# tracel-ai/cubecl

Measured on NVIDIA H100. Metric: bf16_matmul_tflops, higher is better.
Workload: dtype bf16

## Files before the change

cubecl_b200/csrc/gemm_wgmma.cu:

```cuda
#include <cuda_bf16.h>
#include <cuda_fp16.h>

#include "kernel_params.h"
#include "ptx.cuh"

using namespace b200;

enum : int { KIND_F16 = 0, KIND_BF16 = 1, KIND_TF32 = 2, KIND_E4M3 = 3, KIND_E5M2 = 4, KIND_U8 = 5, KIND_S8 = 6 };
enum : int { OUT_F16 = 0, OUT_BF16 = 1, OUT_F32 = 2 };

constexpr int kNumThreads = 384;

#include <type_traits>
struct TileCoord {
  uint32_t b, m_blk, n_blk;
};

__device__ __forceinline__ TileCoord tile_coord(uint32_t t, const GemmParams& p) {
  const uint32_t per_batch = p.tiles_m * p.tiles_n;
  TileCoord c;
  c.b = t / per_batch;
  uint32_t r = t - c.b * per_batch;
  const uint32_t strip = p.group_m * p.tiles_n;
  const uint32_t g = r / strip;
  const uint32_t first_m = g * p.group_m;
  const uint32_t gsize = min(p.group_m, p.tiles_m - first_m);
  const uint32_t in = r - g * strip;
  c.m_blk = first_m + in % gsize;
  c.n_blk = in / gsize;
  return c;
}

struct WorkUnit {
  uint32_t tile, kb0, kb1;
  uint32_t slab;
  bool partial;
};

struct UnitIter {
  uint32_t c, C, num_kb;
  uint32_t r;
  uint32_t u;
  uint64_t pos, hi;
  uint32_t next_tile;
  bool open;
};

__device__ __forceinline__ UnitIter unit_iter(uint32_t cluster, uint32_t n_clusters, uint32_t num_kb) {
  UnitIter it;
  it.c = cluster; it.C = n_clusters; it.num_kb = num_kb;
  it.r = cluster; it.u = 0; it.pos = 0; it.hi = 0; it.next_tile = cluster; it.open = false;
  return it;
}

__device__ __forceinline__ uint64_t sk_range_lo(uint32_t r, const GemmParams& p, uint32_t num_kb) {
  return (static_cast<uint64_t>(r) * p.sk_tiles * num_kb) / p.sk_ranges;
}
__device__ __forceinline__ uint32_t sk_owner(uint64_t x, const GemmParams& p, uint32_t num_kb) {
  return static_cast<uint32_t>(((x + 1) * p.sk_ranges - 1) / (static_cast<uint64_t>(p.sk_tiles) * num_kb));
}

__device__ __forceinline__ bool next_unit(UnitIter& it, const GemmParams& p, WorkUnit& w) {
  while (p.sk_tiles != 0 && it.r < p.sk_ranges) {
    if (!it.open) {
      it.pos = sk_range_lo(it.r, p, it.num_kb);
      it.hi = sk_range_lo(it.r + 1, p, it.num_kb);
      it.u = 0;
      it.open = true;
    }
    if (it.pos < it.hi) {
      const uint32_t tau = static_cast<uint32_t>(it.pos / it.num_kb);
      const uint64_t t0 = static_cast<uint64_t>(tau) * it.num_kb;
      const uint64_t end = (it.hi < t0 + it.num_kb) ? it.hi : t0 + it.num_kb;
      w.tile = p.full_tiles + tau;
      w.kb0 = static_cast<uint32_t>(it.pos - t0);
      w.kb1 = static_cast<uint32_t>(end - t0);
      w.partial = !(w.kb0 == 0 && w.kb1 == it.num_kb);
      w.slab = it.r * p.sk_umax + it.u;
      it.pos = end;
      ++it.u;
      return true;
    }
    it.r += it.C;
    it.open = false;
  }
  if (it.next_tile < p.full_tiles) {
    w.tile = it.next_tile; w.kb0 = 0; w.kb1 = it.num_kb; w.slab = 0; w.partial = false;
    it.next_tile += it.C;
    return true;
  }
  return false;
}


template <int OUT>
__device__ __forceinline__ void store_pair(uint64_t row_ptr, uint32_t n, uint32_t N, bool vec, uint32_t v0, uint32_t v1) {
  if constexpr (OUT == OUT_F32) {
    uint32_t* dst = reinterpret_cast<uint32_t*>(row_ptr) + n;
    if (vec && n + 1 < N) *reinterpret_cast<uint2*>(dst) = make_uint2(v0, v1);
    else { if (n < N) dst[0] = v0; if (n + 1 < N) dst[1] = v1; }
  } else {
    uint16_t* dst = reinterpret_cast<uint16_t*>(row_ptr) + n;
    uint32_t packed;
    if constexpr (OUT == OUT_BF16) asm("cvt.rn.bf16x2.f32 %0, %1, %2;" : "=r"(packed) : "r"(v1), "r"(v0));
    else asm("cvt.rn.f16x2.f32 %0, %1, %2;" : "=r"(packed) : "r"(v1), "r"(v0));
    if (vec && n + 1 < N) *reinterpret_cast<uint32_t*>(dst) = packed;
    else { if (n < N) dst[0] = static_cast<uint16_t>(packed & 0xFFFFu); if (n + 1 < N) dst[1] = static_cast<uint16_t>(packed >> 16); }
  }
}

__device__ __forceinline__ uint32_t acc_bits(float x) { return __float_as_uint(x); }
__device__ __forceinline__ uint32_t acc_bits(uint32_t x) { return x; }

enum : int { QM_NONE = 0, QM_BLOCK = 1, QM_TENSOR = 2 };
enum : int { CB_NONE = 0, CB_DGRAD = 1, CB_WGRAD = 2 };
template <int CG, int BLOCK_N, bool A_MN, bool B_MN, int KIND, int OUT, int STAGES, bool PROMOTE = false, int MT = 1, int QM = QM_NONE,
          bool CONV = false, int CB = CB_NONE>
__device__ __forceinline__ void gemm_body(const CUtensorMap* tma_a_hi, const CUtensorMap* tma_b_hi, const CUtensorMap* tma_a_lo,
                                          const CUtensorMap* tma_b_lo, const CUtensorMap* tma_out, const GemmParams& p) {
  constexpr bool INT_ACC = (KIND == KIND_U8 || KIND == KIND_S8) && QM != QM_BLOCK;
  static_assert(QM == QM_NONE || (KIND == KIND_S8 && !A_MN && !B_MN && !PROMOTE && MT == 1), "quantized operands: s8, K-major");
  static_assert(!CONV || ((KIND == KIND_BF16 || KIND == KIND_F16) && !A_MN && !B_MN && !PROMOTE && MT == 1 && QM == QM_NONE),
                "convolution: 16-bit kinds, K-major operands");
  static_assert(CB != CB_DGRAD || CONV, "data gradient: the convolution producer");
  static_assert(CB != CB_WGRAD || (!CONV && A_MN && B_MN && (KIND == KIND_BF16 || KIND == KIND_F16) && !PROMOTE && MT == 1 && QM == QM_NONE),
                "weight gradient: 16-bit kinds, MN-major operands");
  constexpr uint32_t SC_A_BYTES = (QM == QM_BLOCK) ? 128u * 4u * 4u : 0u;
  constexpr uint32_t SC_STAGE_BYTES = (QM == QM_BLOCK) ? SC_A_BYTES + BLOCK_N * 4u * 4u : 0u;
  constexpr int ESZ = (KIND == KIND_TF32) ? 4 : (KIND >= KIND_E4M3) ? 1 : 2;
  static_assert(ESZ == 2 || (!A_MN && !B_MN), "wgmma reads MN-major operands for 16-bit kinds only");
  constexpr int BLOCK_K = 128 / ESZ;
  constexpr int MMA_K = 32 / ESZ;
  constexpr int N_LOCAL = BLOCK_N / CG;
  constexpr uint32_t A_SUB_BYTES = 128 * 128;
  constexpr uint32_t A_BYTES = MT * A_SUB_BYTES;
  constexpr uint32_t B_BYTES = BLOCK_N * 128;
  constexpr uint32_t STAGE_BYTES = A_BYTES + B_BYTES;
  constexpr int CHUNK_N = 64;
  constexpr uint32_t CHUNK_BYTES = BLOCK_K * 128;
  constexpr int NUM_CHUNKS = N_LOCAL / CHUNK_N;
  constexpr int NACC = BLOCK_N / 2;
  static_assert(STAGE_BYTES % 1024 == 0, "stages must keep 1024-byte alignment for SWIZZLE_128B");
  using Acc = typename std::conditional<INT_ACC, uint32_t, float>::type;
  static_assert(!PROMOTE || (KIND == KIND_BF16 && !A_MN && !B_MN && MT == 1), "promoted accumulation: bf16, K-major operands");
  static_assert(MT == 1 || (MT == 2 && ESZ == 2), "two M sub-tiles per CTA: 16-bit kinds");
  constexpr int PH = (BLOCK_N % 128 == 0) ? 128 : 112;
  static_assert(!PROMOTE || BLOCK_N % PH == 0, "promoted partials tile BLOCK_N");
  constexpr int CW = (OUT == OUT_F32) ? 32 : 64;

  extern __shared__ uint8_t smem_raw[];
  const uint32_t smem_base = (smem_u32(smem_raw) + 1023u) & ~1023u;
  const uint32_t sc_base = smem_base + STAGES * STAGE_BYTES;
  const uint32_t bar_base = sc_base + STAGES * SC_STAGE_BYTES;
  auto full_bar = [&](int s) { return bar_base + 8u * s; };
  auto empty_bar = [&](int s) { return bar_base + 8u * (STAGES + s); };
  const uint32_t split_flag = bar_base + 16u * STAGES;
  const uint32_t epi_base = bar_base + 1024u;

  const uint32_t wg = threadIdx.x >> 7;
  const uint32_t rank = (CG == 2) ? cluster_ctarank() : 0u;
  const uint32_t cluster_id = (CG == 2) ? cluster_id_x() : blockIdx.x;
  const uint32_t n_clusters = (CG == 2) ? num_clusters_x() : gridDim.x;

  if (threadIdx.x == 0) {
    tma_prefetch_desc(tma_a_hi);
    tma_prefetch_desc(tma_b_hi);
    if (p.k_segments > 1) { tma_prefetch_desc(tma_a_lo); tma_prefetch_desc(tma_b_lo); }
    if constexpr (QM == QM_BLOCK) { tma_prefetch_desc(tma_a_lo); tma_prefetch_desc(tma_b_lo); }
    if (p.tma_store) tma_prefetch_desc(tma_out);
    for (int s = 0; s < STAGES; ++s) {
      mbar_init(full_bar(s), 1);
      mbar_init(empty_bar(s), 2 * CG);
    }
    fence_mbar_init();
  }
  if constexpr (CG == 2) cluster_sync_all(); else __syncthreads();

  const uint32_t seg_kb = (p.K + BLOCK_K - 1) / BLOCK_K;
  const bool hyb = (KIND == KIND_TF32) && p.hyb != 0 && p.k_segments == 3;
  const uint32_t seg_kb1 = hyb ? (p.K + 63u) / 64u : seg_kb;
  const uint32_t num_kb = (p.k_segments == 3) ? seg_kb + 2u * seg_kb1 : seg_kb * p.k_segments;
  auto seg_of = [&](uint32_t kb, uint32_t& seg, uint32_t& kk) {
    seg = 0; kk = kb;
    if (kk >= seg_kb) { kk -= seg_kb; seg = 1u + kk / seg_kb1; kk -= (seg - 1u) * seg_kb1; }
  };

  if (wg == 0) {
    setmaxnreg_dec<40>();
    if (threadIdx.x == 0) {
      uint32_t s = 0, ph = 0;
      UnitIter it = unit_iter(cluster_id, n_clusters, num_kb);
      WorkUnit wu;
      while (next_unit(it, p, wu)) {
        const TileCoord tc = tile_coord(wu.tile, p);
        const int m0 = static_cast<int>((tc.m_blk * CG + rank) * (128 * MT));
        const int nb0 = static_cast<int>(tc.n_blk * BLOCK_N);
        const int ba = static_cast<int>(tc.b * p.a_bmul), bb = static_cast<int>(tc.b * p.b_bmul);
        uint32_t seg, kk;
        seg_of(wu.kb0, seg, kk);
        int cv_w = 0, cv_h = 0, cv_n = 0;
        if constexpr (CONV) {
          const uint32_t mu = static_cast<uint32_t>(m0), n = mu / p.cv_ohw, r = mu - n * p.cv_ohw, oh = r / p.cv_ow;
          cv_n = static_cast<int>(n);
          cv_h = static_cast<int>(oh) * p.cv_stride_h - p.cv_pad_h;
          cv_w = static_cast<int>(r - oh * p.cv_ow) * p.cv_stride_w - p.cv_pad_w;
        }
        for (uint32_t kb = wu.kb0; kb < wu.kb1; ++kb) {
          mbar_wait(empty_bar(s), ph ^ 1);
          const uint32_t sa = smem_base + s * STAGE_BYTES;
          const uint32_t sb = sa + A_BYTES;
          const uint32_t fb = full_bar(s);
          if constexpr (CONV) {
            mbar_arrive_expect_tx(fb, STAGE_BYTES);
            const uint32_t kpos = kb / p.cv_cblk, cb = kb - kpos * p.cv_cblk;
            const uint32_t ky = kpos / p.cv_kw, kx = kpos - ky * p.cv_kw;
            const int c0 = static_cast<int>(cb * 64u);
            tma_load_im2col_4d(sa, tma_a_hi, fb, c0, cv_w, cv_h, cv_n, static_cast<uint16_t>(kx * p.cv_dil_w),
                               static_cast<uint16_t>(ky * p.cv_dil_h));
            const int n_row = nb0 + static_cast<int>(rank * N_LOCAL);
            if constexpr (CG == 2) tma_load_3d_mc(sb + rank * N_LOCAL * 128u, tma_b_hi, fb, static_cast<uint16_t>(3), c0, static_cast<int>(kpos), n_row);
            else tma_load_3d(sb, tma_b_hi, fb, c0, static_cast<int>(kpos), n_row);
            if (++s == STAGES) { s = 0; ph ^= 1; }
            continue;
          }
          if constexpr (QM == QM_BLOCK) {
            mbar_arrive_expect_tx(fb, STAGE_BYTES + (128u + BLOCK_N) * 4u * p.q_nsub);
            const uint32_t sc = sc_base + s * SC_STAGE_BYTES;
            const int j0 = static_cast<int>(kk * p.q_nsub);
            tma_load_3d(sc, tma_a_lo, fb, m0, j0, ba);
            tma_load_3d(sc + SC_A_BYTES, tma_b_lo, fb, nb0, j0, bb);
          } else {
            mbar_arrive_expect_tx(fb, STAGE_BYTES);
          }
          auto load_b = [&](uint32_t dst, const CUtensorMap* m, int c0, int c1, int c2) {
            if constexpr (CG == 2) tma_load_3d_mc(dst, m, fb, static_cast<uint16_t>(3), c0, c1, c2);
            else tma_load_3d(dst, m, fb, c0, c1, c2);
          };
          bool h16 = false;
          if constexpr (KIND == KIND_TF32) h16 = hyb && seg != 0;
          if (h16) {
            const int k0 = static_cast<int>(kk * 64u);
            const int ea = ba + static_cast<int>(seg == 2 ? p.hyb_nba : 0u), eb = bb + static_cast<int>(seg == 1 ? p.hyb_nbb : 0u);
            tma_load_3d(sa, tma_a_lo, fb, k0, m0, ea);
            load_b(sb + rank * N_LOCAL * 128u, tma_b_lo, k0, nb0 + static_cast<int>(rank * N_LOCAL), eb);
          } else {
            const int k0 = static_cast<int>(kk * BLOCK_K);
            const CUtensorMap* tma_a = (seg == 2) ? tma_a_lo : tma_a_hi;
            const CUtensorMap* tma_b = (seg == 1) ? tma_b_lo : tma_b_hi;
            if constexpr (A_MN) {
#pragma unroll
              for (int c = 0; c < MT * 128 / CHUNK_N; ++c) tma_load_3d(sa + c * CHUNK_BYTES, tma_a, fb, m0 + c * CHUNK_N, k0, ba);
            } else {
#pragma unroll
              for (int mt = 0; mt < MT; ++mt) tma_load_3d(sa + mt * A_SUB_BYTES, tma_a, fb, k0, m0 + mt * 128, ba);
            }
            if constexpr (CB == CB_WGRAD) {
              const uint32_t px = static_cast<uint32_t>(k0), n = px / p.cv_ohw, r = px - n * p.cv_ohw, oh = r / p.cv_ow;
              const int h = static_cast<int>(oh) * p.cv_stride_h - p.cv_pad_h;
              const int w = static_cast<int>(r - oh * p.cv_ow) * p.cv_stride_w - p.cv_pad_w;
#pragma unroll
              for (int c = 0; c < NUM_CHUNKS; ++c) {
                const int ci = static_cast<int>(rank) * NUM_CHUNKS + c;
                const uint32_t col = min(static_cast<uint32_t>(nb0 + ci * CHUNK_N), p.N - CHUNK_N) / CHUNK_N;
                const uint32_t kpos = col / p.cv_cblk, cb = col - kpos * p.cv_cblk;
                const uint32_t ky = kpos / p.cv_kw, kx = kpos - ky * p.cv_kw;
                const uint16_t ow_ = static_cast<uint16_t>(kx * p.cv_dil_w), oh_ = static_cast<uint16_t>(ky * p.cv_dil_h);
                if constexpr (CG == 2)
                  tma_load_im2col_4d_mc(sb + ci * CHUNK_BYTES, tma_b, fb, static_cast<uint16_t>(3), static_cast<int>(cb * 64u), w, h,
                                        static_cast<int>(n), ow_, oh_);
                else
                  tma_load_im2col_4d(sb + ci * CHUNK_BYTES, tma_b, fb, static_cast<int>(cb * 64u), w, h, static_cast<int>(n), ow_, oh_);
              }
            } else if constexpr (B_MN) {
#pragma unroll
              for (int c = 0; c < NUM_CHUNKS; ++c) {
                const int ci = static_cast<int>(rank) * NUM_CHUNKS + c;
                load_b(sb + ci * CHUNK_BYTES, tma_b, nb0 + ci * CHUNK_N, k0, bb);
              }
            } else {
              load_b(sb + rank * N_LOCAL * 128u, tma_b, k0, nb0 + static_cast<int>(rank * N_LOCAL), bb);
            }
          }
          if (++kk == (seg == 0 ? seg_kb : seg_kb1)) { kk = 0; ++seg; }
          if (++s == STAGES) { s = 0; ph ^= 1; }
        }
      }
    }
  } else {
    setmaxnreg_inc<232>();
    const uint32_t cw = wg - 1;
    const uint32_t ct = threadIdx.x - 128;
    const uint32_t t = threadIdx.x & 127;
    const uint32_t lane = t & 31, wq = t >> 5;
    const uint32_t peer_empty0 = (CG == 2) ? mapa_shared(empty_bar(0), rank ^ 1u) : 0u;
    const bool elected = (t == 0);
    auto release = [&](uint32_t st) {
      if (elected) {
        mbar_arrive(empty_bar(st));
        if constexpr (CG == 2) mbar_arrive_cluster(peer_empty0 + 8u * st);
      }
    };
    const bool mixed = (ESZ == 1) && p.fmt_mixed != 0 && p.fmt_b != ((KIND == KIND_E5M2 || KIND == KIND_S8) ? 1u : 0u);
    constexpr int KIND_OTHER = (KIND == KIND_E4M3) ? KIND_E5M2 : (KIND == KIND_E5M2) ? KIND_E4M3 : (KIND == KIND_U8) ? KIND_S8
                               : (KIND == KIND_S8) ? KIND_U8 : KIND;
    const uint32_t osz = (OUT == OUT_F32) ? 4 : 2;
    float gab = 0.f;
    if constexpr (QM == QM_TENSOR) gab = __fmul_rn(__ldg(reinterpret_cast<const float*>(p.q_ga)), __ldg(reinterpret_cast<const float*>(p.q_gb)));
    Acc acc[MT][NACC];
    uint32_t s = 0, ph = 0;
    UnitIter it = unit_iter(cluster_id, n_clusters, num_kb);
    WorkUnit wu;
    while (next_unit(it, p, wu)) {
      const TileCoord tc = tile_coord(wu.tile, p);
      uint32_t seg = 0, kk = 0;
      if constexpr (KIND == KIND_TF32) seg_of(wu.kb0, seg, kk);
      uint32_t prev = 0;
      if constexpr (PROMOTE || QM == QM_BLOCK) {
#pragma unroll
        for (int i = 0; i < NACC; ++i) acc[0][i] = 0.f;
      }
      for (uint32_t kb = wu.kb0; kb < wu.kb1; ++kb) {
        mbar_wait(full_bar(s), ph);
        const uint32_t sa = smem_base + s * STAGE_BYTES;
        const uint32_t sb = sa + A_BYTES;
        auto a_desc_of = [&](int mt) {
          return A_MN ? make_smem_desc_sw128(sa + (2u * mt + cw) * CHUNK_BYTES, CHUNK_BYTES, 1024)
                      : make_smem_desc_sw128(sa + mt * A_SUB_BYTES + cw * 64u * 128u, 16, 1024);
        };
        const uint64_t a_desc = a_desc_of(0);
        const uint64_t b_desc = B_MN ? make_smem_desc_sw128(sb, CHUNK_BYTES, 1024) : make_smem_desc_sw128(sb, 16, 1024);
        if constexpr (PROMOTE) {
          float part[PH / 2];
#pragma unroll
          for (int h = 0; h < BLOCK_N / PH; ++h) {
            wgmma_fence();
#pragma unroll
            for (int k = 0; k < 4; ++k)
              wgmma_ss<PH, KIND_BF16, KIND_BF16, 0, 0>(part, a_desc + 2 * k, b_desc + ((h * PH * 128u) >> 4) + 2 * k, k != 0 ? 1u : 0u);
            wgmma_commit();
            wgmma_wait<0>();
            wgmma_fence_operands(part);
#pragma unroll
            for (int i = 0; i < PH / 2; ++i) acc[0][PH / 2 * h + i] += part[i];
          }
          release(s);
        } else if constexpr (QM == QM_BLOCK) {
          const uint32_t sc = sc_base + s * SC_STAGE_BYTES;
          const uint32_t row = cw * 64u + wq * 16u + (lane >> 2);
          auto fold_stage = [&](auto ns) {
            constexpr uint32_t NSUB = decltype(ns)::value, KPER = 4u / NSUB;
#pragma unroll
            for (uint32_t j = 0; j < NSUB; ++j) {
              float ra0, ra1;
              asm volatile("ld.shared.f32 %0, [%1];" : "=f"(ra0) : "r"(sc + (j * 128u + row) * 4u) : "memory");
              asm volatile("ld.shared.f32 %0, [%1];" : "=f"(ra1) : "r"(sc + (j * 128u + row + 8u) * 4u) : "memory");
              const uint32_t scb = sc + SC_A_BYTES + (j * BLOCK_N + 2u * (lane & 3u)) * 4u;
#pragma unroll
              for (int h = 0; h < BLOCK_N / 64; ++h) {
                uint32_t part[32];
                wgmma_fence();
#pragma unroll
                for (uint32_t k = 0; k < KPER; ++k) {
                  const uint32_t kk2 = 2u * (j * KPER + k);
                  wgmma_ss<64, KIND_S8, KIND_S8, 0, 0>(part, a_desc + kk2, b_desc + ((h * 64u * 128u) >> 4) + kk2, k != 0 ? 1u : 0u);
                }
                wgmma_commit();
                wgmma_wait<0>();
                wgmma_fence_operands(part);
#pragma unroll
                for (int g = 0; g < 8; ++g) {
                  float cb0, cb1;
                  asm volatile("ld.shared.v2.f32 {%0, %1}, [%2];" : "=f"(cb0), "=f"(cb1) : "r"(scb + (h * 64u + 8u * g) * 4u) : "memory");
                  const float sc4[4] = {__fmul_rn(ra0, cb0), __fmul_rn(ra0, cb1), __fmul_rn(ra1, cb0), __fmul_rn(ra1, cb1)};
#pragma unroll
                  for (int e = 0; e < 4; ++e) {
                    const float d = __fsub_rn(__int_as_float(static_cast<int>(part[4 * g + e]) + 0x4B400000), 12582912.f);
                    acc[0][32 * h + 4 * g + e] = __fmaf_rn(d, sc4[e], acc[0][32 * h + 4 * g + e]);
                  }
                }
              }
            }
          };
          if (p.q_nsub == 4) fold_stage(std::integral_constant<uint32_t, 4>{});
          else if (p.q_nsub == 2) fold_stage(std::integral_constant<uint32_t, 2>{});
          else fold_stage(std::integral_constant<uint32_t, 1>{});
          release(s);
        } else {
  #pragma unroll
          for (int mt = 0; mt < MT; ++mt) wgmma_fence_operands(acc[mt]);
          wgmma_fence();
          bool h16 = false;
          if constexpr (KIND == KIND_TF32) {
            h16 = hyb && seg != 0;
            if (++kk == (seg == 0 ? seg_kb : seg_kb1)) { kk = 0; ++seg; }
          }
          if (h16) {
            if constexpr (KIND == KIND_TF32) {
  #pragma unroll
              for (int k = 0; k < 4; ++k)
                wgmma_ss<BLOCK_N, KIND_BF16, KIND_BF16, 0, 0>(acc[0], a_desc + 2 * k, b_desc + 2 * k, (kb != wu.kb0 || k != 0) ? 1u : 0u);
            }
          } else if (mixed) {
            if constexpr (ESZ == 1) {
  #pragma unroll
              for (int k = 0; k < BLOCK_K / MMA_K; ++k)
                wgmma_ss<BLOCK_N, KIND, KIND_OTHER, 0, 0>(acc[0], a_desc + 2 * k, b_desc + 2 * k, (kb != wu.kb0 || k != 0) ? 1u : 0u);
            }
          } else {
  #pragma unroll
            for (int k = 0; k < BLOCK_K / MMA_K; ++k) {
              const uint64_t b_k = b_desc + static_cast<uint64_t>(B_MN ? ((k * MMA_K * 128) >> 4) : 2 * k);
  #pragma unroll
              for (int mt = 0; mt < MT; ++mt) {
                const uint64_t a_k = a_desc_of(mt) + static_cast<uint64_t>(A_MN ? ((k * MMA_K * 128) >> 4) : 2 * k);
                wgmma_ss<BLOCK_N, KIND, KIND, A_MN ? 1 : 0, B_MN ? 1 : 0>(acc[mt], a_k, b_k, (kb != wu.kb0 || k != 0) ? 1u : 0u);
              }
            }
          }
          wgmma_commit();
          if (kb != wu.kb0) {
            wgmma_wait<1>();
            release(prev);
          }
  #pragma unroll
          for (int mt = 0; mt < MT; ++mt) wgmma_fence_operands(acc[mt]);
          prev = s;
        }
        if (++s == STAGES) { s = 0; ph ^= 1; }
      }
      if constexpr (!PROMOTE && QM != QM_BLOCK) {
        wgmma_wait<0>();
#pragma unroll
        for (int mt = 0; mt < MT; ++mt) wgmma_fence_operands(acc[mt]);
        release(prev);
      }

      const uint32_t m_cta = (tc.m_blk * CG + rank) * (128u * MT);
      const uint32_t c0 = tc.n_blk * BLOCK_N + 2u * (lane & 3u);
      auto epilogue = [&](uint32_t n, uint32_t (&v)[4]) {
        if (!INT_ACC && QM == QM_NONE && p.epi_on) {
          const float* bias = reinterpret_cast<const float*>(p.bias);
#pragma unroll
          for (int e = 0; e < 4; ++e) {
            const uint32_t col = n + (e & 1);
            float x = __uint_as_float(v[e]) * p.alpha;
            if (bias != nullptr && col < p.N) x += __ldg(bias + col);
            if (p.epi_act == 1) x = fmaxf(x, 0.f);
            else if (p.epi_act == 2) x = 0.5f * x * (1.f + erff(x * 0.70710678118654752f));
            v[e] = __float_as_uint(x);
          }
        }
      };
      uint64_t dg_row[2] = {0, 0};
      if constexpr (CB == CB_DGRAD) {
#pragma unroll
        for (int h = 0; h < 2; ++h) {
          const uint32_t r = m_cta + cw * 64u + wq * 16u + (lane >> 2) + 8u * h;
          const uint32_t n = r / p.cv_ohw, rr = r - n * p.cv_ohw, i = rr / p.cv_ow, j = rr - i * p.cv_ow;
          dg_row[h] = p.out + (n * p.dx_sn + i * p.dx_si + j * p.dx_sj) * osz;
        }
      }
      auto store_group = [&](int mt, int j, uint32_t (&v)[4]) {
        const uint32_t n = c0 + 8u * j;
        if (n >= p.N) return;
        epilogue(n, v);
        const uint32_t r0 = m_cta + mt * 128u + cw * 64u + wq * 16u + (lane >> 2);
        if constexpr (CB == CB_DGRAD) {
          if (r0 < p.M) store_pair<OUT>(dg_row[0], n, p.N, p.vec_store != 0, v[0], v[1]);
          if (r0 + 8 < p.M) store_pair<OUT>(dg_row[1], n, p.N, p.vec_store != 0, v[2], v[3]);
        } else if constexpr (CB == CB_WGRAD) {
          const uint32_t kpos = n / (p.cv_cblk * 64u), ch = n - kpos * p.cv_cblk * 64u;
          const uint64_t row0 = p.out + (static_cast<uint64_t>(r0) * p.out_row_stride + kpos * p.dw_sp) * osz;
          if (r0 < p.M) store_pair<OUT>(row0, ch, p.dw_c, p.vec_store != 0, v[0], v[1]);
          if (r0 + 8 < p.M) store_pair<OUT>(row0 + static_cast<uint64_t>(8) * p.out_row_stride * osz, ch, p.dw_c, p.vec_store != 0, v[2], v[3]);
        } else {
          const uint64_t row0 = p.out + (static_cast<uint64_t>(tc.b) * p.out_batch_stride + static_cast<uint64_t>(r0) * p.out_row_stride) * osz;
          if (r0 < p.M) store_pair<OUT>(row0, n, p.N, p.vec_store != 0, v[0], v[1]);
          if (r0 + 8 < p.M) store_pair<OUT>(row0 + static_cast<uint64_t>(8) * p.out_row_stride * osz, n, p.N, p.vec_store != 0, v[2], v[3]);
        }
      };
      auto frag = [&](int mt, int j, uint32_t (&v)[4]) {
#pragma unroll
        for (int e = 0; e < 4; ++e) {
          if constexpr (QM == QM_TENSOR) v[e] = __float_as_uint(__fmul_rn(__int2float_rn(static_cast<int>(acc[mt][4 * j + e])), gab));
          else v[e] = acc_bits(acc[mt][4 * j + e]);
        }
      };
      const bool partial = (MT == 1) && !INT_ACC && QM == QM_NONE && wu.partial;

      if (CB != CB_DGRAD && !partial && p.tma_store) {
        const uint32_t stage_smem = epi_base + cw * 8192u;
        const uint32_t rl = wq * 16u + (lane >> 2);
#pragma unroll
        for (int mt = 0; mt < MT; ++mt) {
          const int m_row0 = static_cast<int>(m_cta + mt * 128u + cw * 64u);
#pragma unroll
          for (int c = 0; c < BLOCK_N / CW; ++c) {
            const uint32_t n0 = tc.n_blk * BLOCK_N + c * CW;
            if (t == 0) tma_store_wait_read<0>();
            asm volatile("bar.sync %0, 128;" ::"r"(2u + cw) : "memory");
#pragma unroll
            for (int jj = 0; jj < CW / 8; ++jj) {
              const int j = c * (CW / 8) + jj;
              uint32_t v[4];
              frag(mt, j, v);
              epilogue(c0 + 8u * j, v);
              const uint32_t cb = (8u * jj + 2u * (lane & 3u)) * osz;
#pragma unroll
              for (int h = 0; h < 2; ++h) {
                const uint32_t r = rl + 8u * h;
                const uint32_t addr = stage_smem + r * 128u + ((((cb >> 4) ^ (r & 7u)) << 4) | (cb & 15u));
                if constexpr (OUT == OUT_F32) {
                  asm volatile("st.shared.v2.b32 [%0], {%1, %2};" ::"r"(addr), "r"(v[2 * h]), "r"(v[2 * h + 1]) : "memory");
                } else {
                  uint32_t packed;
                  if constexpr (OUT == OUT_BF16) asm("cvt.rn.bf16x2.f32 %0, %1, %2;" : "=r"(packed) : "r"(v[2 * h + 1]), "r"(v[2 * h]));
                  else asm("cvt.rn.f16x2.f32 %0, %1, %2;" : "=r"(packed) : "r"(v[2 * h + 1]), "r"(v[2 * h]));
                  asm volatile("st.shared.b32 [%0], %1;" ::"r"(addr), "r"(packed) : "memory");
                }
              }
            }
            fence_proxy_async_smem();
            asm volatile("bar.sync %0, 128;" ::"r"(2u + cw) : "memory");
            if (t == 0 && m_row0 < static_cast<int>(p.M) && n0 < p.N) {
              if constexpr (CB == CB_WGRAD) {
                const uint32_t kpos = n0 / (p.cv_cblk * 64u);
                tma_store_3d(tma_out, stage_smem, static_cast<int>(n0 - kpos * p.cv_cblk * 64u), m_row0, static_cast<int>(kpos));
              } else {
                tma_store_3d(tma_out, stage_smem, static_cast<int>(n0), m_row0, static_cast<int>(tc.b));
              }
              tma_store_commit();
            }
          }
#pragma unroll
          for (int j = BLOCK_N / CW * CW / 8; j < NACC / 4; ++j) {
            uint32_t v[4];
            frag(mt, j, v);
            store_group(mt, j, v);
          }
        }
      } else if (!partial) {
#pragma unroll
        for (int mt = 0; mt < MT; ++mt) {
#pragma unroll
          for (int j = 0; j < NACC / 4; ++j) {
            uint32_t v[4];
            frag(mt, j, v);
            store_group(mt, j, v);
          }
        }
      } else {
        const uint64_t cta_slab_bytes = static_cast<uint64_t>(128) * BLOCK_N * 4;
        uint4* dst = reinterpret_cast<uint4*>(p.split_ws + (static_cast<uint64_t>(wu.slab) * CG + rank) * cta_slab_bytes) + ct;
#pragma unroll
        for (int j = 0; j < NACC / 4; ++j)
          __stcg(dst + j * 256, make_uint4(acc_bits(acc[0][4 * j]), acc_bits(acc[0][4 * j + 1]), acc_bits(acc[0][4 * j + 2]), acc_bits(acc[0][4 * j + 3])));
        const uint32_t tau = wu.tile - p.full_tiles;
        const uint32_t first = sk_owner(static_cast<uint64_t>(tau) * num_kb, p, num_kb);
        const uint32_t parts = sk_owner(static_cast<uint64_t>(tau + 1) * num_kb - 1, p, num_kb) - first + 1;
        __threadfence();
        asm volatile("bar.sync 1, 256;" ::: "memory");
        if (ct == 0) {
          unsigned int* ticket = reinterpret_cast<unsigned int*>(p.split_tickets) + tau * CG + rank;
          const unsigned int old = atomicAdd(ticket, 1u);
          const uint32_t last = (old == parts - 1) ? 1u : 0u;
          if (last) *ticket = 0;
          asm volatile("st.shared.u32 [%0], %1;" ::"r"(split_flag), "r"(last) : "memory");
        }
        asm volatile("bar.sync 1, 256;" ::: "memory");
        uint32_t last;
        asm volatile("ld.shared.u32 %0, [%1];" : "=r"(last) : "r"(split_flag) : "memory");
        if (last) {
          __threadfence();
          auto part_slab = [&](uint32_t j) {
            const uint32_t r = first + j;
            const uint32_t u = tau - static_cast<uint32_t>(sk_range_lo(r, p, num_kb) / num_kb);
            return reinterpret_cast<const float4*>(p.split_ws + ((static_cast<uint64_t>(r) * p.sk_umax + u) * CG + rank) * cta_slab_bytes) + ct;
          };
#pragma unroll 1
          for (int j = 0; j < NACC / 4; ++j) {
            float4 sum = make_float4(0.f, 0.f, 0.f, 0.f);
            for (uint32_t sl = 0; sl < parts; ++sl) {
              const float4 x = __ldcg(part_slab(sl) + j * 256);
              sum.x += x.x; sum.y += x.y; sum.z += x.z; sum.w += x.w;
            }
            uint32_t v[4] = {__float_as_uint(sum.x), __float_as_uint(sum.y), __float_as_uint(sum.z), __float_as_uint(sum.w)};
            store_group(0, j, v);
          }
        }
        asm volatile("bar.sync 1, 256;" ::: "memory");
      }
    }
    if (t == 0) tma_store_wait<0>();
  }

  if constexpr (CG == 2) cluster_sync_all(); else __syncthreads();
}


#define GEMM_KERNEL_PM(NAME, CG, BN, AMN, BMN, KIND, OUT, STAGES, PROMOTE, MT)                                     \
  extern "C" __global__ void __launch_bounds__(kNumThreads, 1)                                                     \
      NAME(const __grid_constant__ CUtensorMap tma_a, const __grid_constant__ CUtensorMap tma_b,                  \
           const __grid_constant__ CUtensorMap tma_a_lo, const __grid_constant__ CUtensorMap tma_b_lo,            \
           const __grid_constant__ CUtensorMap tma_out, const __grid_constant__ GemmParams p) {                    \
    gemm_body<CG, BN, AMN, BMN, KIND, OUT, STAGES, PROMOTE, MT>(&tma_a, &tma_b, &tma_a_lo, &tma_b_lo, &tma_out, p); \
  }
#define GEMM_KERNEL_P(NAME, CG, BN, AMN, BMN, KIND, OUT, STAGES, PROMOTE) GEMM_KERNEL_PM(NAME, CG, BN, AMN, BMN, KIND, OUT, STAGES, PROMOTE, 1)
#define GEMM_KERNEL(NAME, CG, BN, AMN, BMN, KIND, OUT, STAGES) GEMM_KERNEL_P(NAME, CG, BN, AMN, BMN, KIND, OUT, STAGES, false)

#define GEMM_LAYOUTS(PFX, CG, BN, KIND, OUT, STAGES)           \
  GEMM_KERNEL(PFX##_kn, CG, BN, false, true, KIND, OUT, STAGES)  \
  GEMM_KERNEL(PFX##_kk, CG, BN, false, false, KIND, OUT, STAGES) \
  GEMM_KERNEL(PFX##_mn, CG, BN, true, true, KIND, OUT, STAGES)   \
  GEMM_KERNEL(PFX##_mk, CG, BN, true, false, KIND, OUT, STAGES)
#define GEMM_DTYPES(TILE, CG, BN, STAGES)                                                  \
  GEMM_LAYOUTS(gemm_bf16_bf16_##TILE, CG, BN, KIND_BF16, OUT_BF16, STAGES)                  \
  GEMM_LAYOUTS(gemm_bf16_f32_##TILE, CG, BN, KIND_BF16, OUT_F32, STAGES)                    \
  GEMM_LAYOUTS(gemm_f16_f16_##TILE, CG, BN, KIND_F16, OUT_F16, STAGES)                      \
  GEMM_LAYOUTS(gemm_f16_f32_##TILE, CG, BN, KIND_F16, OUT_F32, STAGES)                      \
  GEMM_LAYOUTS(gemm_f16_bf16_##TILE, CG, BN, KIND_F16, OUT_BF16, STAGES)                    \
  GEMM_KERNEL(gemm_tf32_f32_##TILE##_kk, CG, BN, false, false, KIND_TF32, OUT_F32, STAGES)
#define GEMM_INT8(TILE, CG, BN, STAGES)                                                      \
  GEMM_KERNEL(gemm_u8_i32_##TILE##_kk, CG, BN, false, false, KIND_U8, OUT_F32, STAGES)        \
  GEMM_KERNEL(gemm_s8_i32_##TILE##_kk, CG, BN, false, false, KIND_S8, OUT_F32, STAGES)
#define GEMM_MX(TILE, CG, BN, STAGES)                                                                     \
  GEMM_KERNEL_P(gemm_mx_bf16_##TILE##_kk, CG, BN, false, false, KIND_BF16, OUT_BF16, STAGES, true)         \
  GEMM_KERNEL_P(gemm_mx_f16_##TILE##_kk, CG, BN, false, false, KIND_BF16, OUT_F16, STAGES, true)           \
  GEMM_KERNEL_P(gemm_mx_f32_##TILE##_kk, CG, BN, false, false, KIND_BF16, OUT_F32, STAGES, true)

#define GEMM_KERNEL_Q(NAME, CG, BN, OUT, STAGES, QM)                                                                  \
  extern "C" __global__ void __launch_bounds__(kNumThreads, 1)                                                     \
      NAME(const __grid_constant__ CUtensorMap tma_a, const __grid_constant__ CUtensorMap tma_b,                  \
           const __grid_constant__ CUtensorMap tma_a_sc, const __grid_constant__ CUtensorMap tma_b_sc,            \
           const __grid_constant__ CUtensorMap tma_out, const __grid_constant__ GemmParams p) {                    \
    gemm_body<CG, BN, false, false, KIND_S8, OUT, STAGES, false, 1, QM>(&tma_a, &tma_b, &tma_a_sc, &tma_b_sc, &tma_out, p); \
  }
#define GEMM_Q8T(TILE, CG, BN, STAGES)                                                     \
  GEMM_KERNEL_Q(gemm_q8t_bf16_##TILE##_kk, CG, BN, OUT_BF16, STAGES, QM_TENSOR)            \
  GEMM_KERNEL_Q(gemm_q8t_f16_##TILE##_kk, CG, BN, OUT_F16, STAGES, QM_TENSOR)              \
  GEMM_KERNEL_Q(gemm_q8t_f32_##TILE##_kk, CG, BN, OUT_F32, STAGES, QM_TENSOR)
#define GEMM_Q(TILE, CG, BN, STAGES, QSTAGES)                                              \
  GEMM_KERNEL_Q(gemm_q8_bf16_##TILE##_kk, CG, BN, OUT_BF16, QSTAGES, QM_BLOCK)             \
  GEMM_KERNEL_Q(gemm_q8_f16_##TILE##_kk, CG, BN, OUT_F16, QSTAGES, QM_BLOCK)               \
  GEMM_KERNEL_Q(gemm_q8_f32_##TILE##_kk, CG, BN, OUT_F32, QSTAGES, QM_BLOCK)               \
  GEMM_Q8T(TILE, CG, BN, STAGES)

#define CONV_KERNEL(NAME, CG, BN, KIND, OUT, STAGES)                                                                \
  extern "C" __global__ void __launch_bounds__(kNumThreads, 1)                                                     \
      NAME(const __grid_constant__ CUtensorMap tma_a, const __grid_constant__ CUtensorMap tma_b,                  \
           const __grid_constant__ CUtensorMap tma_a_lo, const __grid_constant__ CUtensorMap tma_b_lo,            \
           const __grid_constant__ CUtensorMap tma_out, const __grid_constant__ GemmParams p) {                    \
    gemm_body<CG, BN, false, false, KIND, OUT, STAGES, false, 1, QM_NONE, true>(&tma_a, &tma_b, &tma_a_lo, &tma_b_lo, &tma_out, p); \
  }
#define CONV_DTYPES(TILE, CG, BN, STAGES)                                  \
  CONV_KERNEL(conv2d_bf16_bf16_##TILE, CG, BN, KIND_BF16, OUT_BF16, STAGES) \
  CONV_KERNEL(conv2d_bf16_f32_##TILE, CG, BN, KIND_BF16, OUT_F32, STAGES)   \
  CONV_KERNEL(conv2d_f16_f16_##TILE, CG, BN, KIND_F16, OUT_F16, STAGES)     \
  CONV_KERNEL(conv2d_f16_f32_##TILE, CG, BN, KIND_F16, OUT_F32, STAGES)

#define CONV_BWD_KERNEL(NAME, CG, BN, AMN, KIND, OUT, STAGES, CONV, CB)                                            \
  extern "C" __global__ void __launch_bounds__(kNumThreads, 1)                                                     \
      NAME(const __grid_constant__ CUtensorMap tma_a, const __grid_constant__ CUtensorMap tma_b,                  \
           const __grid_constant__ CUtensorMap tma_a_lo, const __grid_constant__ CUtensorMap tma_b_lo,            \
           const __grid_constant__ CUtensorMap tma_out, const __grid_constant__ GemmParams p) {                    \
    gemm_body<CG, BN, AMN, AMN, KIND, OUT, STAGES, false, 1, QM_NONE, CONV, CB>(&tma_a, &tma_b, &tma_a_lo, &tma_b_lo, &tma_out, p); \
  }
#define CONV_BWD_DTYPES(TILE, CG, BN, STAGES)                                                                  \
  CONV_BWD_KERNEL(conv2d_dgrad_bf16_bf16_##TILE, CG, BN, false, KIND_BF16, OUT_BF16, STAGES, true, CB_DGRAD)   \
  CONV_BWD_KERNEL(conv2d_dgrad_bf16_f32_##TILE, CG, BN, false, KIND_BF16, OUT_F32, STAGES, true, CB_DGRAD)     \
  CONV_BWD_KERNEL(conv2d_dgrad_f16_f16_##TILE, CG, BN, false, KIND_F16, OUT_F16, STAGES, true, CB_DGRAD)       \
  CONV_BWD_KERNEL(conv2d_dgrad_f16_f32_##TILE, CG, BN, false, KIND_F16, OUT_F32, STAGES, true, CB_DGRAD)       \
  CONV_BWD_KERNEL(conv2d_wgrad_bf16_bf16_##TILE, CG, BN, true, KIND_BF16, OUT_BF16, STAGES, false, CB_WGRAD)   \
  CONV_BWD_KERNEL(conv2d_wgrad_bf16_f32_##TILE, CG, BN, true, KIND_BF16, OUT_F32, STAGES, false, CB_WGRAD)     \
  CONV_BWD_KERNEL(conv2d_wgrad_f16_f16_##TILE, CG, BN, true, KIND_F16, OUT_F16, STAGES, false, CB_WGRAD)       \
  CONV_BWD_KERNEL(conv2d_wgrad_f16_f32_##TILE, CG, BN, true, KIND_F16, OUT_F32, STAGES, false, CB_WGRAD)

#ifndef GEMM_PART
#define GEMM_PART 0
#endif

#if GEMM_PART == 0
GEMM_DTYPES(2sm_n256, 2, 256, 4)
GEMM_INT8(2sm_n256, 2, 256, 4)
GEMM_MX(2sm_n256, 2, 256, 4)
#endif
#if GEMM_PART == 1
GEMM_DTYPES(2sm_n128, 2, 128, 6)
GEMM_INT8(2sm_n128, 2, 128, 6)
GEMM_MX(2sm_n128, 2, 128, 6)
GEMM_MX(2sm_n224, 2, 224, 4)
#endif
#if GEMM_PART == 2
GEMM_DTYPES(1sm_n128, 1, 128, 6)
GEMM_INT8(1sm_n128, 1, 128, 6)
GEMM_MX(1sm_n128, 1, 128, 6)
#define GEMM_M512(PFX, KIND, OUT)                                                     \
  GEMM_KERNEL_PM(PFX##_2sm_m512_kn, 2, 128, false, true, KIND, OUT, 4, false, 2)       \
  GEMM_KERNEL_PM(PFX##_2sm_m512_kk, 2, 128, false, false, KIND, OUT, 4, false, 2)      \
  GEMM_KERNEL_PM(PFX##_2sm_m512_mn, 2, 128, true, true, KIND, OUT, 4, false, 2)        \
  GEMM_KERNEL_PM(PFX##_2sm_m512_mk, 2, 128, true, false, KIND, OUT, 4, false, 2)
GEMM_M512(gemm_bf16_bf16, KIND_BF16, OUT_BF16)
GEMM_M512(gemm_bf16_f32, KIND_BF16, OUT_F32)
GEMM_M512(gemm_f16_f16, KIND_F16, OUT_F16)
GEMM_M512(gemm_f16_f32, KIND_F16, OUT_F32)
GEMM_M512(gemm_f16_bf16, KIND_F16, OUT_BF16)
#endif
#if GEMM_PART == 3
GEMM_Q8T(2sm_n256, 2, 256, 4)
GEMM_Q(2sm_n128, 2, 128, 6, 5)
GEMM_Q(1sm_n128, 1, 128, 6, 5)
#endif
#if GEMM_PART == 4
CONV_DTYPES(2sm_n128, 2, 128, 6)
CONV_DTYPES(1sm_n128, 1, 128, 6)
#endif
#if GEMM_PART == 5
CONV_BWD_DTYPES(2sm_n128, 2, 128, 6)
CONV_BWD_DTYPES(1sm_n128, 1, 128, 6)
#endif

#if GEMM_PART == 0
template <int PK>
__device__ __forceinline__ void wgmma_probe_body(float* out, uint32_t n_iter) {
  extern __shared__ uint8_t smem_probe_raw[];
  const uint32_t smem_base = (smem_u32(smem_probe_raw) + 1023u) & ~1023u;
  const uint32_t sa = smem_base, sb = smem_base + 16384;
  const uint32_t ones = PK == 0 ? 0x3F803F80u : 0x38383838u;
  for (uint32_t i = threadIdx.x; i < (16384 + 32768) / 4; i += blockDim.x)
    asm volatile("st.shared.u32 [%0], %1;" ::"r"(smem_base + 4 * i), "r"(ones) : "memory");
  fence_proxy_async_smem();
  __syncthreads();
  const uint32_t wg = threadIdx.x >> 7;
  if (wg == 0) return;
  float acc[128];
  const uint64_t a_desc = make_smem_desc_sw128(sa + (wg - 1) * 8192u, 16, 1024), b_desc = make_smem_desc_sw128(sb, 16, 1024);
  for (uint32_t i = 0; i < n_iter; ++i) {
    wgmma_fence();
#pragma unroll
    for (int k = 0; k < 4; ++k) {
      if constexpr (PK == 0) wgmma_ss<256, KIND_BF16, KIND_BF16, 0, 0>(acc, a_desc + 2 * k, b_desc + 2 * k, (i | k) != 0 ? 1u : 0u);
      else wgmma_ss<256, KIND_E4M3, KIND_E4M3, 0, 0>(acc, a_desc + 2 * k, b_desc + 2 * k, (i | k) != 0 ? 1u : 0u);
    }
    wgmma_commit();
  }
  wgmma_wait<0>();
  wgmma_fence_operands(acc);
  if (threadIdx.x == 128) out[blockIdx.x] = acc[0];
}
extern "C" __global__ void __launch_bounds__(384, 1) wgmma_probe_bf16(float* out, uint32_t n_iter) { wgmma_probe_body<0>(out, n_iter); }
extern "C" __global__ void __launch_bounds__(384, 1) wgmma_probe_e4m3(float* out, uint32_t n_iter) { wgmma_probe_body<1>(out, n_iter); }
#endif
```

Before: 564.7.

## Stage whole output tile in the last pipeline stage buffer for TMA store

In the common bf16/f16 non-split case, the consumer no longer releases the final pipeline stage after the mainloop. It writes the entire swizzled output tile into that stage buffer (spilling into the epilogue staging area), issues all TMA stores at once, and only releases the stage at the start of the next tile's mainloop after the stores have finished reading. This removes the per-chunk wait-and-barrier cycle of the old staged epilogue so that stores overlap with the next tile's loads. The cost is that the producer runs with one fewer free stage during that window, and the correctness depends on the stage-index bookkeeping and the barrier usage.

```diff
diff --git a/cubecl_b200/csrc/gemm_wgmma.cu b/cubecl_b200/csrc/gemm_wgmma.cu
--- a/cubecl_b200/csrc/gemm_wgmma.cu
+++ b/cubecl_b200/csrc/gemm_wgmma.cu
@@ -147,6 +147,8 @@
   constexpr int PH = (BLOCK_N % 128 == 0) ? 128 : 112;
   static_assert(!PROMOTE || BLOCK_N % PH == 0, "promoted partials tile BLOCK_N");
   constexpr int CW = (OUT == OUT_F32) ? 32 : 64;
+  constexpr bool BORROW = MT == 1 && !PROMOTE && QM == QM_NONE && !CONV && CB == CB_NONE && OUT != OUT_F32;
+  static_assert(!BORROW || (BLOCK_N % 64 == 0 && 256u * BLOCK_N <= STAGE_BYTES + 16384u), "a 16-bit tile fits a stage + staging");
 
   extern __shared__ uint8_t smem_raw[];
   const uint32_t smem_base = (smem_u32(smem_raw) + 1023u) & ~1023u;
@@ -308,6 +310,7 @@
     if constexpr (QM == QM_TENSOR) gab = __fmul_rn(__ldg(reinterpret_cast<const float*>(p.q_ga)), __ldg(reinterpret_cast<const float*>(p.q_gb)));
     Acc acc[MT][NACC];
     uint32_t s = 0, ph = 0;
+    bool held = false;
     UnitIter it = unit_iter(cluster_id, n_clusters, num_kb);
     WorkUnit wu;
     while (next_unit(it, p, wu)) {
@@ -421,6 +424,12 @@
           if (kb != wu.kb0) {
             wgmma_wait<1>();
             release(prev);
+          } else if constexpr (BORROW) {
+            if (held) {
+              if (elected) tma_store_wait_read<0>();
+              release(s == 0 ? STAGES - 1 : s - 1);
+              held = false;
+            }
           }
   #pragma unroll
           for (int mt = 0; mt < MT; ++mt) wgmma_fence_operands(acc[mt]);
@@ -432,7 +441,7 @@
         wgmma_wait<0>();
 #pragma unroll
         for (int mt = 0; mt < MT; ++mt) wgmma_fence_operands(acc[mt]);
-        release(prev);
+        if (!(BORROW && !wu.partial && p.tma_store)) release(prev);
       }
 
       const uint32_t m_cta = (tc.m_blk * CG + rank) * (128u * MT);
@@ -488,7 +497,45 @@
       };
       const bool partial = (MT == 1) && !INT_ACC && QM == QM_NONE && wu.partial;
 
-      if (CB != CB_DGRAD && !partial && p.tma_store) {
+      if (BORROW && !partial && p.tma_store) {
+        const uint32_t tile_smem = smem_base + prev * STAGE_BYTES;
+        auto chunk_smem = [&](uint32_t q) { return q * 8192u < STAGE_BYTES ? tile_smem + q * 8192u : epi_base + (q * 8192u - STAGE_BYTES); };
+        const uint32_t rl = wq * 16u + (lane >> 2);
+        asm volatile("bar.sync 1, 256;" ::: "memory");
+#pragma unroll
+        for (int c = 0; c < BLOCK_N / 64; ++c) {
+          const uint32_t chunk = chunk_smem(cw * (BLOCK_N / 64) + c);
+#pragma unroll
+          for (int jj = 0; jj < 8; ++jj) {
+            const int j = c * 8 + jj;
+            uint32_t v[4];
+            frag(0, j, v);
+            epilogue(c0 + 8u * j, v);
+            const uint32_t cb = (8u * jj + 2u * (lane & 3u)) * 2u;
+#pragma unroll
+            for (int h = 0; h < 2; ++h) {
+              const uint32_t r = rl + 8u * h;
+              const uint32_t addr = chunk + r * 128u + ((((cb >> 4) ^ (r & 7u)) << 4) | (cb & 15u));
+              uint32_t packed;
+              if constexpr (OUT == OUT_BF16) asm("cvt.rn.bf16x2.f32 %0, %1, %2;" : "=r"(packed) : "r"(v[2 * h + 1]), "r"(v[2 * h]));
+              else asm("cvt.rn.f16x2.f32 %0, %1, %2;" : "=r"(packed) : "r"(v[2 * h + 1]), "r"(v[2 * h]));
+              asm volatile("st.shared.b32 [%0], %1;" ::"r"(addr), "r"(packed) : "memory");
+            }
+          }
+        }
+        fence_proxy_async_smem();
+        asm volatile("bar.sync %0, 128;" ::"r"(2u + cw) : "memory");
+        const int m_row0 = static_cast<int>(m_cta + cw * 64u);
+        if (t == 0 && m_row0 < static_cast<int>(p.M)) {
+#pragma unroll
+          for (int c = 0; c < BLOCK_N / 64; ++c) {
+            const uint32_t n0 = tc.n_blk * BLOCK_N + c * 64;
+            if (n0 < p.N) tma_store_3d(tma_out, chunk_smem(cw * (BLOCK_N / 64) + c), static_cast<int>(n0), m_row0, static_cast<int>(tc.b));
+          }
+          tma_store_commit();
+        }
+        held = true;
+      } else if (CB != CB_DGRAD && !partial && p.tma_store) {
         const uint32_t stage_smem = epi_base + cw * 8192u;
         const uint32_t rl = wq * 16u + (lane >> 2);
 #pragma unroll
```

Measured after the change: 544.8, median of 6. 0.965x the previous value.
